# adolliou/euispice_coreg

Hardware: AMD Instinct MI355X
Metric: lag-points/sec (whole node) on 2048² grid, 60×60 CRVAL sweep; argmax-shift match (higher is better)
Workload: dtype f64; 1 GPU; headline: Carrington 'fa' 2048x2048 grid lon(200,300) lat(-20,20), 60x60 CRVAL lags arange(-30,30,1) arcsec, small 2048^2 HRIEUV-like, ref 3072^2 FSI-like, order 2, solar_r 1.004; lag_points=3600, parallelism=single GPU, no collective, resident=True, sweeps_in_flight=2, small_stored_f32=True, use_lds=True

## Files before the change

### euispice_coreg_amd/csrc/abi_sweeps.hpp

```cpp
#pragma once
namespace {
struct SweepCall {
    const coreg_lags* lags = nullptr;
    LagDims d;
    int order = 0, method = 0, sem = 0;
    long long lag_begin = 0, lag_end = 0, n_out = 0;
    double* corr_out = nullptr;
    int out_on_device = 0;
    double* out_dev = nullptr;
    long long row() const { return (long long)d.n2 * d.nc; }
    int i1_lo() const { return (int)(lag_begin / row()); }
    int i1_hi() const { return (int)((lag_end - 1) / row()); }
};

template <typename OwnChecks>
int open_sweep(coreg_handle* h, ComboRange combo, OwnChecks own_checks, const coreg_lags* lags, int order, int method,
               int sem, int64_t lag_begin, int64_t lag_end, int grid_w, int grid_h, const char* grid_what,
               double* corr_out, int out_on_device, SweepCall* call) {
    if (method != COREG_METHOD_CORRELATION && method != COREG_METHOD_RESIDUS && method != COREG_METHOD_RESIDUS_MASKED)
        return fail(h, COREG_ENOTIMPL,
                    "method must be COREG_METHOD_CORRELATION, COREG_METHOD_RESIDUS or COREG_METHOD_RESIDUS_MASKED");
    RETCHK(check_order(h, order));
    RETCHK(own_checks());
    RETCHK(check_lags(h, lags, &call->d, lag_begin, lag_end, combo));
// ... 9 lines not shown
    call->n_out = lag_end - lag_begin;
    call->corr_out = corr_out;
    call->out_on_device = out_on_device;
    return begin_sweep(h, call->n_out, corr_out, out_on_device, &call->out_dev);
}

int close_sweep(coreg_handle* h, const SweepCall& call) {
    return end_sweep(h, call.n_out, call.corr_out, call.out_on_device, call.out_dev);
}

int close_empty_sweep(coreg_handle* h, const SweepCall& call) {
    RETCHK(fill_nan(h, call.out_dev, call.n_out));
    RETCHK(fill_nan(h, h->counts.as<double>(), call.n_out));
    return close_sweep(h, call);
}

template <typename MapAt>
Geometry local_geometry(const coreg_wcs2d& target, const SweepCall& call, MapAt at) {
    const coreg_lags& l = *call.lags;
    int e1[3], e2[3];
    extreme_lags(l.crval1, call.d.n1, e1);
    extreme_lags(l.crval2, call.d.n2, e2);
    const double v1 = l.crval1[e1[1]], v2 = l.crval2[e2[1]];
    const double s1 = lag_step(l.crval1, call.d.n1), s2 = lag_step(l.crval2, call.d.n2);
    const double u = target.naxis1 * 0.5, v = target.naxis2 * 0.5;
    double x0, y0, xi, yi, xj, yj, xa, ya, xb, yb;
    Geometry g;
    if (!at(v1, v2, u, v, &x0, &y0) || !at(v1, v2, u + 1, v, &xi, &yi) || !at(v1, v2, u, v + 1, &xj, &yj) ||
        !at(v1 + s1, v2, u, v, &xa, &ya) || !at(v1, v2 + s2, u, v, &xb, &yb))
        return g;
    g.dx_di = xi - x0;
    g.dy_di = yi - y0;
    g.dx_dj = xj - x0;
    g.dy_dj = yj - y0;
    g.ax = xa - x0;
    g.ay = ya - y0;
    g.bx = xb - x0;
    g.by = yb - y0;
    return g;
}

Plan plan_sweep(coreg_handle* h, const Geometry& geo, const SweepCall& call) {
    return choose_plan(h, geo, call.i1_hi() - call.i1_lo() + 1, call.d.n2, h->opt_use_lds ? lds_window_elems(h) : (1LL << 40));
}

bool combo_slots(const SweepCall& call, const coreg_wcs2d& small, const Plan& plan, long long c, coreg_wcs2d* hc,
                 SlotList* slots) {
    const long long first = (call.lag_begin - c + call.d.nc - 1) / call.d.nc;
    if (first * call.d.nc + c >= call.lag_end) return false;
    int i3, i4, i5;
    call.d.inner(c, &i3, &i4, &i5);
    if (shift_header(small, 0.0, 0.0, call.lags->cdelt1[i3], call.lags->cdelt2[i4], call.lags->crota[i5], call.sem, hc))
        return false;
    build_slots(call.d, c, call.lag_begin, call.lag_end, plan.sw, plan.sh, slots);
    return slots->n_batches > 0;
}

template <int MODE>
int precompute(coreg_handle* h, const PrecomputeArgs& pa, int n_tiles, int n_groups, int n_batches, bool launch = true) {
    if (launch) RETCHK(launch_precompute<MODE>(h, pa, n_tiles, n_groups, n_batches));
    h->last_precompute = [pa, n_tiles, n_groups, n_batches](coreg_handle* hh) {
        return launch_precompute<MODE>(hh, pa, n_tiles, n_groups, n_batches);
    };
    return COREG_OK;
}

SweepLaunchSpec sweep_launch(const SweepCall& call, int mode, size_t slot_off, int n_batches, int n_tiles) {
    SweepLaunchSpec sl;
    sl.mode = mode;
    sl.order = call.order;
    sl.method = call.method;
    sl.slot_off = slot_off;
    sl.n_batches = n_batches;
    sl.n_tiles = n_tiles;
    sl.lag_begin = call.lag_begin;
    sl.out_dev = call.out_dev;
    return sl;
}

int finalize_pending(coreg_handle* h, const coreg_handle::PendingFinalize& pf, long long* refine_count, double* out_dev,
                     FinalizeArgs* f) {
    *f = FinalizeArgs{};
    RETCHK(fill_refine(h, &f->refine, pf.refine.mode, pf.refine.order, pf.refine.lane_params, pf.refine.car_inv,
                       pf.n_slots));
    f->refine.enabled = pf.refine.enabled;
    f->refine_count = refine_count;
    f->partials = h->sums.as<double>() + pf.slot_off;
    f->n_groups = 1;
    f->n_slots = pf.n_slots;
    f->part_stride = h->sums_slots;
    f->out_index = h->fin_outidx.as<long long>() + pf.slot_off;
    f->lag_begin = pf.lag_begin;
    f->out = out_dev;
    f->counts = h->counts.as<double>();
    f->residus = pf.residus;
    f->n_required = (long long)h->gW * h->gH;
    launch_finalize(h, *f);
    return COREG_OK;
}
}

extern "C" {
int coreg_sweep_carrington(coreg_handle* h, const coreg_wcs2d* hdr_small, const coreg_carr_grid* grid, double solar_r,
                           const coreg_lags* lags, int order, int method, int cdelt_semantics, int64_t lag_begin,
                           int64_t lag_end, double* corr_out, int out_on_device) {
    if (!h) return COREG_EINVAL;
    const ComboRange combo = take_combo_range(h);
// ... 636 lines not shown
```

### euispice_coreg_amd/csrc/coreg_hip.hip

```cpp
#include <hip/hip_runtime.h>

#include <algorithm>
#include <chrono>
#include <cmath>
#include <cstdio>
#include <cstdlib>
#include <cstring>
#include <limits>
#include <condition_variable>
#include <map>
#include <memory>
#include <mutex>
#include <string>
#include <thread>
#include <functional>
#include <type_traits>
#include <utility>
#include <vector>

#include "fit.hpp"
#include "geometry.hpp"
#include "kernels.hpp"
#include <atomic>
#include "ricecomp.hpp"
#include "riceenc.hpp"

using namespace coreg;

#define COREG_VERSION "0.1.0"

#include "host_state.hpp"
#include "host_upload.hpp"
#include "host_plan.hpp"
#include "host_fix_launch.hpp"
#include "sweep_variant.hpp"
#include "host_sweep_launch.hpp"
#include "host_fix_lists.hpp"
#include "host_sweep_io.hpp"
#include "host_context.hpp"
#include "host_pixels.hpp"


extern "C" {

const char* coreg_version(void) { return "coreg_hip " COREG_VERSION " (gfx950)"; }

int coreg_create(coreg_handle** out, int device) {
    if (!out) return COREG_EINVAL;
    *out = nullptr;
    coreg_handle* h = new (std::nothrow) coreg_handle();
    if (!h) return COREG_ENOMEM;
    int ndev = 0;
    hipError_t e = hipGetDeviceCount(&ndev);
    if (e != hipSuccess || ndev < 1) {
        delete h;
        return COREG_EHIP;
    }
    if (device < 0) {
        if (hipGetDevice(&device) != hipSuccess) device = 0;
    }
    if (device >= ndev) {
        delete h;
        return COREG_EINVAL;
    }
    h->device = device;
    if (hipSetDevice(device) != hipSuccess || hipStreamCreateWithFlags(&h->stream, hipStreamNonBlocking) != hipSuccess ||
        hipEventCreate(&h->ev_end[0]) != hipSuccess ||
        hipEventCreate(&h->ev_end[1]) != hipSuccess || hipEventRecord(h->ev_end[0], h->stream) != hipSuccess ||
        hipEventRecord(h->ev_end[1], h->stream) != hipSuccess ||
        h->pivots.reserve(2 * sizeof(double)) != hipSuccess ||
        hipMemsetAsync(h->pivots.p, 0, 2 * sizeof(double), h->stream) != hipSuccess) {
        h->own_stream = h->stream != nullptr;
        coreg_destroy(h);
        return COREG_EHIP;
    }
    h->own_stream = true;
    std::memset(&h->stats, 0, sizeof(h->stats));
    *out = h;
    return COREG_OK;
}

void coreg_destroy(coreg_handle* h) {
    if (!h) return;
// ... 164 lines not shown
```

### euispice_coreg_amd/csrc/host_plan.hpp

```cpp
#pragma once
namespace {
template <typename Fn>
void parallel_for(long long n, unsigned max_threads, long long grain, Fn fn) {
    if (n <= 0) return;
    const long long nt_max = std::max<long long>(1, std::min(max_threads, std::thread::hardware_concurrency()));
    if (grain <= 0) grain = (n + nt_max - 1) / nt_max;
    const long long nt = std::min(nt_max, (n + grain - 1) / grain);
    if (nt <= 1) {
        fn(0ll, n);
        return;
    }
    std::atomic<long long> next(0);
    auto worker = [&] {
        for (long long lo = next.fetch_add(grain); lo < n; lo = next.fetch_add(grain)) fn(lo, std::min(n, lo + grain));
    };
    std::vector<std::thread> th;
    for (long long t = 1; t < nt; ++t) th.emplace_back(worker);
    worker();
    for (auto& x : th) x.join();
}

struct LagDims {
    int n1, n2, n3, n4, n5;
    long long nc;
    long long c0;
    long long total() const { return (long long)n1 * n2 * nc; }
    void inner(long long c, int* i3, int* i4, int* i5) const {
        const long long g = c + c0;
        *i5 = (int)(g % n5);
        *i4 = (int)((g / n5) % n4);
        *i3 = (int)(g / ((long long)n5 * n4));
    }
};

struct ComboRange {
    long long begin = 0, end = 0;
};
ComboRange take_combo_range(coreg_handle* h) {
    ComboRange r;
    r.begin = h->opt_combo_begin;
    r.end = h->opt_combo_end;
    h->opt_combo_begin = h->opt_combo_end = 0;
    return r;
}
int check_lags(coreg_handle* h, const coreg_lags* l, LagDims* d, int64_t begin, int64_t end, ComboRange combo = ComboRange()) {
    if (!l || !l->crval1 || !l->crval2 || !l->cdelt1 || !l->cdelt2 || !l->crota)
        return fail(h, COREG_EINVAL, "lags: null array");
    if (l->n_crval1 < 1 || l->n_crval2 < 1 || l->n_cdelt1 < 1 || l->n_cdelt2 < 1 || l->n_crota < 1)
        return fail(h, COREG_EINVAL, "lags: every axis needs at least one value");
    d->n1 = l->n_crval1;
    d->n2 = l->n_crval2;
    d->n3 = l->n_cdelt1;
    d->n4 = l->n_cdelt2;
    d->n5 = l->n_crota;
    d->nc = (long long)d->n3 * d->n4 * d->n5;
    d->c0 = 0;
    {
        const long long cb = combo.begin, ce = combo.end;
        if (cb != 0 || ce != 0) {
            if (cb < 0 || ce <= cb || ce > d->nc)
                return fail(h, COREG_EINVAL, "combo_begin/combo_end outside [0, n_cdelt1 * n_cdelt2 * n_crota]");
            d->c0 = cb;
            d->nc = ce - cb;
        }
    }
    if (begin < 0 || end > d->total() || begin > end)
        return fail(h, COREG_EINVAL, "lag_begin/lag_end outside [0, n_lags]");
    const double* ax[5] = {l->crval1, l->crval2, l->cdelt1, l->cdelt2, l->crota};
    const int32_t na[5] = {l->n_crval1, l->n_crval2, l->n_cdelt1, l->n_cdelt2, l->n_crota};
    for (int k = 0; k < 5; ++k)
        for (int32_t i = 0; i < na[k]; ++i)
            if (!std::isfinite(ax[k][i])) return fail(h, COREG_EINVAL, "lags: a non-finite value");
    return COREG_OK;
}

static int check_wcs(coreg_handle* h, const coreg_wcs2d* w, bool carrington_transform) {
    const char* why = wcs_problem(*w, carrington_transform);
    return why ? fail(h, COREG_EINVAL, why) : COREG_OK;
}
static int check_grid(coreg_handle* h, const coreg_carr_grid* g) {
    if (g->n_lon >= 1 && g->n_lat >= 1 && too_many(g->n_lon, g->n_lat))
        return fail(h, COREG_EINVAL, "Carrington grid: more than 2^31 - 1 points");
    const char* why = grid_problem(*g);
    return why ? fail(h, COREG_EINVAL, why) : COREG_OK;
}

struct Geometry {
    double dx_di = 1, dx_dj = 0, dy_di = 0, dy_dj = 1;
    double ax = 0, ay = 0, bx = 0, by = 0;
};
struct Plan {
    int tile_w = 32;
    int sw = 16, sh = 16;
    double window = 0;
    double win_w = 0, win_h = 0;
};

Plan choose_plan(coreg_handle* h, const Geometry& g, int m1, int n2, long long lds_elems) {
    Plan best, fallback;
    double best_cost = std::numeric_limits<double>::max(), fb_win = std::numeric_limits<double>::max();
    const int sw_hi = h->opt_patch_w > 0 ? std::min<int>((int)h->opt_patch_w, kBlock) : kBlock;
    for (int tw = 4; tw <= 256; tw *= 2) {
        if (h->opt_tile_w > 0 && tw != h->opt_tile_w) continue;
        const int th = kTilePts / tw;
        if (th < 1) continue;
        const double tex = tw * std::fabs(g.dx_di) + th * std::fabs(g.dx_dj);
        const double tey = tw * std::fabs(g.dy_di) + th * std::fabs(g.dy_dj);
        for (int sw = 1; sw <= std::min(m1, sw_hi); ++sw) {
            int sh = std::min(n2, kBlock / sw);
            if (sh < 1) break;
            const int cols = (m1 + sw - 1) / sw, rows = (n2 + sh - 1) / sh;
            sh = (n2 + rows - 1) / rows;
            const int sw2 = (m1 + cols - 1) / cols;
            const double ex = tex + sw2 * std::fabs(g.ax) + sh * std::fabs(g.bx) + 6.0;
            const double ey = tey + sw2 * std::fabs(g.ay) + sh * std::fabs(g.by) + 6.0;
            const double win = (ex + 1.0) * ey;
            if (win < fb_win) {
                fb_win = win;
                fallback.tile_w = tw;
                fallback.sw = sw2;
                fallback.sh = sh;
                fallback.window = win;
                fallback.win_w = ex + 1.0;
                fallback.win_h = ey;
            }
            if (win > 0.94 * (double)lds_elems) continue;
            const double cost = (double)cols * rows * (1.0 + 0.08 * win / (double)lds_elems);
            if (cost < best_cost) {
                best_cost = cost;
                best.tile_w = tw;
                best.sw = sw2;
                best.sh = sh;
                best.window = win;
                best.win_w = ex + 1.0;
                best.win_h = ey;
            }
        }
    }
    const Plan& r = best_cost < std::numeric_limits<double>::max() ? best : fallback;
    if (std::getenv("COREG_DEBUG_PLAN"))
        std::fprintf(stderr, "[coreg plan] tile %d x %d, lag patch %d x %d, window estimate %.0f (%.1f x %.1f) of %lld elements; "
                     "geometry d/di (%.3f, %.3f) d/dj (%.3f, %.3f) lag1 (%.3f, %.3f) lag2 (%.3f, %.3f)\n", r.tile_w,
                     kTilePts / r.tile_w, r.sw, r.sh, r.window, r.win_w, r.win_h, lds_elems, g.dx_di, g.dy_di, g.dx_dj, g.dy_dj, g.ax, g.ay,
                     g.bx, g.by);
    return r;
}

void extreme_lags(const double* v, int n, int out[3]) {
    int lo = 0, hi = 0;
    for (int i = 1; i < n; ++i) {
        if (v[i] < v[lo] || v[lo] != v[lo]) lo = i;
        if (v[i] > v[hi] || v[hi] != v[hi]) hi = i;
    }
    const double mid = 0.5 * (v[lo] + v[hi]);
    int m = lo;
    for (int i = 0; i < n; ++i)
        if (std::fabs(v[i] - mid) < std::fabs(v[m] - mid)) m = i;
    out[0] = lo;
    out[1] = m;
    out[2] = hi;
}

double lag_step(const double* v, int n) {
    if (n < 2) return 0.0;
    double lo = v[0], hi = v[0];
    for (int i = 1; i < n; ++i) {
        lo = std::min(lo, v[i]);
        hi = std::max(hi, v[i]);
    }
    return (hi - lo) / (double)(n - 1);
}

struct SlotList {
    std::vector<int> i1, i2;
    std::vector<long long> outidx;
    int n_batches = 0;
};

void build_slots(const LagDims& d, long long c, long long begin, long long end, int sw, int sh, SlotList* s) {
    s->i1.clear();
    s->i2.clear();
    s->outidx.clear();
    s->n_batches = 0;
    {
        const size_t cap = (size_t)((d.n1 + sw - 1) / sw + 1) * ((d.n2 + sh - 1) / sh) * kBlock;
        s->i1.reserve(cap);
        s->i2.reserve(cap);
        s->outidx.reserve(cap);
    }
    const long long row = (long long)d.n2 * d.nc;
    const int i1_lo = (int)(begin / row);
    const int i1_hi = (int)((end - 1) / row);
    const int m1 = i1_hi - i1_lo + 1;
    for (int p1 = 0; p1 * sw < m1; ++p1)
        for (int p2 = 0; p2 * sh < d.n2; ++p2) {
            bool any = false;
            const size_t at = s->i1.size();
            for (int t = 0; t < kBlock; ++t) {
                int lx = t % sw, ly = t / sw;
                bool valid = ly < sh;
                if (!valid) lx = ly = 0;
                int i1 = i1_lo + p1 * sw + lx, i2 = p2 * sh + ly;
                if (i1 > i1_hi) {
                    i1 = i1_hi;
                    valid = false;
                }
                if (i2 > d.n2 - 1) {
                    i2 = d.n2 - 1;
                    valid = false;
                }
                const long long idx = ((long long)i1 * d.n2 + i2) * d.nc + c;
                if (idx < begin || idx >= end) valid = false;
                s->i1.push_back(i1);
                s->i2.push_back(i2);
                s->outidx.push_back(valid ? idx : -1);
                any |= valid;
            }
            if (!any) {
                s->i1.resize(at);
                s->i2.resize(at);
                s->outidx.resize(at);
            } else {
                s->n_batches++;
            }
        }
}

int pick_groups(coreg_handle* h, int n_batches, int n_tiles) {
    if (h->opt_shard_world > 1) {
        const long long per_rank = 8 * std::max<long long>(1, std::llround(256.0 / (8.0 * n_batches)));
        return (int)std::min<long long>(per_rank * h->opt_shard_world, 1000 / (8 * h->opt_shard_world) * 8 * h->opt_shard_world);
    }
    long long g = h->opt_n_groups > 0 ? h->opt_n_groups : (4096 + n_batches - 1) / n_batches;
    (void)n_tiles;
    g = std::max<long long>(8, std::min<long long>(h->opt_n_groups > 0 ? 1000 : 256, ((g + 7) / 8) * 8));
    return (int)g;
}

void pick_taper(const coreg_handle* h, int n_groups, int n_batches, int* tmin, int* tfrac) {
    *tmin = (int)h->opt_taper_min;
    if (h->opt_taper_frac >= 0) {
        *tfrac = (int)h->opt_taper_frac;
        return;
    }
    const double rounds = (double)n_groups * n_batches / 256.0;
    *tfrac = (rounds >= (double)h->opt_taper_rounds && n_groups >= 128 && h->opt_shard_world <= 1) ? 512 : 0;
}

template <int MODE>
int launch_precompute(coreg_handle* h, const PrecomputeArgs& a, int n_tiles, int n_groups, int n_batches) {
    EventPair* ev = next_event(h, h->ev_pre, h->ev_pre_used);
    if (!ev) return fail(h, COREG_EHIP, "hipEventCreate failed");
    int tmin, tfrac;
    pick_taper(h, n_groups, n_batches, &tmin, &tfrac);
    PrecomputeArgs b = a;
    b.prologue = h->pending_prologue;
    const bool with_prologue = b.prologue.src != nullptr;
    std::memset(&h->pending_prologue, 0, sizeof(h->pending_prologue));
    HIPCHK(hipEventRecord(ev->a, h->stream));
    if (h->ref_dtype == COREG_F32)
        hipLaunchKernelGGL((k_precompute<MODE, float>), dim3(n_tiles), dim3(256), 0, h->stream, b);
    else
        hipLaunchKernelGGL((k_precompute<MODE, double>), dim3(n_tiles), dim3(256), 0, h->stream, b);
    (void)with_prologue;
    hipLaunchKernelGGL(k_tile_list, dim3(1), dim3(1024), 0, h->stream, (const int*)a.tile_count, n_tiles, n_groups,
                       h->tile_list.as<int>(), h->tile_cum.as<int>(), h->group_first.as<int>(),
                       h->tile_info.as<long long>(), tmin, tfrac);
    ev->b_is_next_sweep = true;
    ev->next_sweep_index = h->ev_sweep_used;
    HIPCHK(hipGetLastError());
    return COREG_OK;
}

int reserve_tiles(coreg_handle* h, int n_tiles) {
    const size_t pts = (size_t)n_tiles * kTilePts + (size_t)(kPointGroups + 1) * kChunk;
    HIPCHK(h->pts.reserve(pts * sizeof(Pt)));
    HIPCHK(h->tile_count.reserve(n_tiles * sizeof(int)));
    HIPCHK(h->tile_list.reserve(n_tiles * sizeof(int)));
    HIPCHK(h->tile_cum.reserve((n_tiles + 1) * sizeof(int)));
    HIPCHK(h->group_first.reserve(2 * 1024 * sizeof(int) + 64));
    HIPCHK(h->tile_info.reserve(8 * sizeof(long long)));
    HIPCHK(h->tile_bbox.reserve((size_t)n_tiles * 4 * sizeof(double)));
    return COREG_OK;
}

int setup_precompute(coreg_handle* h, const Plan& plan, int method, PrecomputeArgs* a, int* n_tiles) {
    std::memset(a, 0, sizeof(*a));
    a->tile_w = plan.tile_w;
    a->tile_h = kTilePts / plan.tile_w;
    a->tiles_x = (h->gW + a->tile_w - 1) / a->tile_w;
    a->tiles_y = (h->gH + a->tile_h - 1) / a->tile_h;
    *n_tiles = a->tiles_x * a->tiles_y;
    RETCHK(reserve_tiles(h, *n_tiles));
    a->ref = h->ref.p;
    a->gw = h->gW;
    a->gh = h->gH;
    a->pivot_a = h->pivots.as<double>();
    a->pts = h->pts.as<Pt>();
    a->tile_count = h->tile_count.as<int>();
    a->tile_bbox = h->tile_bbox.as<double>();
    a->residus = method != COREG_METHOD_CORRELATION ? 1 : 0;
    return COREG_OK;
}

long long lds_window_elems(const coreg_handle* h);

int pick_pitch(const coreg_handle* h, const Plan& plan, long long lds_elems, int order = 2) {
    if (h->opt_pitch == 0 || !h->opt_use_lds) return 0;
    static const int kPitches[] = {89, 121, 153, 185, 217};
    if (h->opt_pitch > 0) {
        for (int p : kPitches)
            if (p == h->opt_pitch) return p;
        return 0;
    }
    for (int p : kPitches)
        if ((double)p >= plan.win_w + (order > 2 ? 4.0 : 2.0) &&
            (double)p * (plan.win_h + (order > 2 ? 2.0 : 0.0)) <= 0.985 * (double)lds_elems)
            return p;
    return 0;
}

}
```

### euispice_coreg_amd/csrc/host_state.hpp

```cpp
#pragma once
namespace {

struct DevBuf {
    void* p = nullptr;
    size_t cap = 0;
    hipError_t reserve(size_t bytes) {
        if (bytes <= cap) return hipSuccess;
        if (p) {
            hipError_t e = hipFree(p);
            if (e != hipSuccess) return e;
            p = nullptr;
            cap = 0;
        }
        const size_t want = bytes + bytes / 4 + 256;
        hipError_t e = hipMalloc(&p, want);
        if (e != hipSuccess) return e;
        cap = want;
        return hipSuccess;
    }
    void release() {
        if (p) (void)hipFree(p);
        p = nullptr;
        cap = 0;
    }
// ... 100 lines not shown
    std::vector<double> tabs_key;
    PinBuf pin_img[2];
    hipEvent_t ev_img[2] = {nullptr, nullptr};
    int pin_img_next = 0;
    DevBuf pts, tile_count, tile_list, tile_cum, group_first, tile_info, tile_bbox;
    DevBuf rf_fix_slab;
    DevBuf counters;
    DevBuf lane_params, out_index, partials, out_dev, tmp_img;
    DevBuf counts;
    long long counts_n = -1;
    DevBuf up_f64, up_flag;
    DevBuf up_raw;
    DevBuf rice_blob, rice_rand, dec_img;
    PrologueArgs pending_prologue = {};
    DevBuf bbox_buf;
    hipStream_t aux_stream = nullptr;
    hipStream_t up_stream = nullptr;
    hipEvent_t ev_small = nullptr, ev_main = nullptr;
    bool small_pending = false;
    DevBuf red_sum_up, red_cnt_up;
    int64_t opt_overlap_upload = 1;
    int64_t opt_tap_nan_filter = 2;
    int64_t opt_async_upload = 0;
    std::thread up_thread;
    std::mutex up_m;
    std::condition_variable up_cv;
    std::function<hipError_t()> up_job;
    bool up_has = false, up_stop = false, up_busy = false;
    hipError_t up_rc = hipSuccess;
    PinBuf pin_small[2];
    hipEvent_t ev_pin_small[2] = {nullptr, nullptr};
    int pin_small_next = 0;
    std::map<std::vector<double>, std::vector<int>> border_cache;
    std::map<std::vector<double>, std::vector<unsigned char>> flags_cache;
    DevBuf border_flags, fix_partial;
    DevBuf border_dev;
    PinBuf pin_border;
    int64_t opt_border_fix = 1;
    int64_t opt_tap_fix = 1, opt_tap_cap = 1 << 24;
    DevBuf tap_count, tap_segq, tap_list, tap_skip, tap_seg_slot, tap_seg_begin, tap_pixel, tap_xw, tap_yw;
    long long tap_last[3] = {0, 0, 0};
    int64_t opt_shard_world = 1, opt_shard_rank = 0;
    int64_t opt_combo_begin = 0, opt_combo_end = 0;
    DevBuf sums;
    long long sums_slots = 0;
    struct PendingFinalize {
        long long slot_off, n_slots, lag_begin;
        int residus;
        RefineArgs refine;
        std::function<int(coreg_handle*)> replay_precompute;
        FixLaunch fixes;
    };
    std::function<int(coreg_handle*)> last_precompute;
    DevBuf rf_flags, rf_pivots, rf_list, rf_head, rf_partial;
    std::vector<PendingFinalize> pending_fin;
    DevBuf fin_outidx;
    long long pending_n_out = 0;

    int64_t opt_crop_reference = 1;
    int64_t opt_taper_min = 128, opt_taper_frac = -1, opt_taper_rounds = 6;
    int64_t opt_use_lds = 1, opt_clean_path = 1, opt_refine = 1, opt_refine_cond_log10 = 5, opt_tile_w = 0, opt_n_groups = 0, opt_lds_bytes = (159 * 1024 * kPointGroups) / 4, opt_patch_w = 0, opt_h_series = 1, opt_h_incr = 1, opt_tile_skip = 1, opt_pitch = -1;

    coreg_stats stats;
    bool stats_pending = false;
    PinBuf pin_info;
    std::vector<EventPair> ev_sweep, ev_pre;
    size_t ev_sweep_used = 0, ev_pre_used = 0;
    hipEvent_t ev_t1 = nullptr;
    hipEvent_t ev_end[2] = {nullptr, nullptr};
    PinBuf pin_plan[2];
    int plan_slot = 0;
    bool plan_open = false;
};
```

### euispice_coreg_amd/csrc/kernels_sweep.hpp

```cpp
#pragma once
namespace coreg {
struct SweepArgs {
    const void* img;
    int W, H;
    const Pt* pts;
    const int* tile_count;
    const int* tile_list;
    const int* tile_cum;
    const int* group_first;
    long long* tile_info;
    const double* tile_bbox;
    const double* lane_params;
    long long n_slots;
    int n_batches;
    int n_groups;
    int group_lo;
    double* partials;
    const double* pivots;
    int use_lds;
    int clean_path;
    int lds_elems;
    LaunchU car_inv;
};

// ... 500 lines not shown
                    cur = nxt;
                }
            }
        }
    }
#else
    for (int c = p_begin / kChunk + pg; c < n_full; c += kPointGroups) {
        const Pt* __restrict__ q = pts + c * kChunk;
        Pt pt[kChunk];
#pragma unroll
        for (int k = 0; k < kChunk; ++k) load_pt_uniform(q + k, pt[k]);
#pragma unroll
        for (int k = 0; k < kChunk; ++k)
            point_lag<MODE, ORDER, TS, LDS, ROUND, RESID, INTERIOR, PITCH, CLEAN>(acc, win, img, pitch, ox, oy, W, H, wmax,
                                                                                  hmax, px0, py0, pxw, pyw, hm, cu, pt[k].b0,
                                                                                  pt[k].b1, pt[k].a, pt[k].pad, pivot_b);
        if constexpr (CLEAN) {
            acc.n += kChunk;
            acc.a += pt[1].pad;
            acc.aa += pt[2].pad;
        }
    }
#endif
    if (pg == n_full % kPointGroups) {
        for (int p = n_full * kChunk; p < p_end; ++p) {
            Pt pt;
            load_pt_uniform(pts + p, pt);
            point_lag<MODE, ORDER, TS, LDS, ROUND, RESID, INTERIOR, PITCH>(acc, win, img, pitch, ox, oy, W, H, wmax, hmax,
                                                                           px0, py0, pxw, pyw, hm, cu, pt.b0, pt.b1, pt.a,
                                                                           pt.pad, pivot_b);
        }
    }
}

template <int MODE, int ORDER, typename TS, bool ROUND, bool RESID, int PITCH = 0>
__global__ void __launch_bounds__(kSweepThreads) k_sweep(const SweepArgs a) {
    extern __shared__ __align__(16) unsigned char lds_raw[];
    double* lds = (double*)lds_raw;
    constexpr int kWaves = kSweepThreads / 64;
    constexpr int kLagWaves = kBlock / 64;
    __shared__ double wred2[2][kLagWaves][4];
    __shared__ int wdirty[2][kWaves];
    constexpr bool kCleanPath = MODE != MODE_CAR && !RESID && ORDER != ORDER_RT && !(ROUND && sizeof(TS) == 8);
    int visit = 0;
    int n_vis = 0, n_vis_lds = 0, n_vis_int = 0, n_vis_clean = 0;

    const int b = blockIdx.x;
    const int slot8 = b & 7;
    const int q = b >> 3;
    const int batch = q % a.n_batches;
    const int group = a.group_lo + (q / a.n_batches) * 8 + slot8;

    const int lane = threadIdx.x & 63, wave = threadIdx.x >> 6;
    const int pg = __builtin_amdgcn_readfirstlane(threadIdx.x / kBlock);
    const long long slot = (long long)batch * kBlock + (threadIdx.x % kBlock);

    double px0 = 0.0, py0 = 0.0;
    H9 hm;
#pragma unroll
    for (int k = 0; k < 9; ++k) hm.h[k] = 0.0;
    if (MODE == MODE_TRANSLATE) {
        px0 = a.lane_params[slot];
        py0 = a.lane_params[a.n_slots + slot];
    } else {
#pragma unroll
        for (int k = 0; k < 9; ++k) hm.h[k] = a.lane_params[(long long)k * a.n_slots + slot];
    }

    const bool pad_lane = MODE == MODE_TRANSLATE ? (px0 != px0) : (hm.h[8] != hm.h[8]);

    Acc acc = {0, 0.0, 0.0, 0.0, 0.0, 0.0};

    const TS* __restrict__ img = (const TS*)a.img;
    const int W = a.W, H = a.H;
    const double inf = __builtin_inf();
    const int u_lo = a.group_first[1024 + group];
    const int u_hi = a.group_first[1024 + group + 1];
    const int n_list = (int)a.tile_info[0];
    const double pivot_b = a.pivots[1];
#if defined(__HIP_DEVICE_COMPILE__)
    const unsigned win = (unsigned)(uintptr_t)(__attribute__((address_space(3))) unsigned char*)lds_raw;
#else
    const unsigned win = 0;
#endif

    for (int tl = a.group_first[group]; tl < n_list && u_lo < u_hi; ++tl) {
        const int ubase = a.tile_cum[tl];
        if (ubase >= u_hi) break;
        const int tile = a.tile_list[tl];
        const int cnt = a.tile_count[tile];
        const int p_begin = max(u_lo - ubase, 0) * kUnitPts;
        const int p_end = min((u_hi - ubase) * kUnitPts, cnt);
        if (p_begin >= p_end) continue;
        const double* bb = a.tile_bbox + (size_t)tile * 4;
        const double bx0 = bb[0], bx1 = bb[1], by0 = bb[2], by1 = bb[3];

        double mnx, mxx, mny, mxy;
        if (MODE == MODE_TRANSLATE) {
            mnx = bx0 + px0;
            mxx = bx1 + px0;
            mny = by0 + py0;
            mxy = by1 + py0;
        } else {
            mnx = inf; mxx = -inf; mny = inf; mxy = -inf;
#pragma unroll
            for (int c = 0; c < 4; ++c) {
                double cx, cy;
                apply_map<MODE>(hm, a.car_inv, (c & 1) ? bx1 : bx0, (c & 2) ? by1 : by0, cx, cy);
                mnx = fmin(mnx, cx);
                mxx = fmax(mxx, cx);
                mny = fmin(mny, cy);
                mxy = fmax(mxy, cy);
            }
            if (MODE == MODE_CAR) {
                const double margin = car_tile_margin(a.car_inv.box_c, fmax(fabs(by0), fabs(by1)) + a.car_inv.pole_sep);
                mnx -= margin;
                mxx += margin;
                mny -= margin;
                mxy += margin;
            }
        }
        for (int o = 32; o > 0; o >>= 1) {
            mnx = fmin(mnx, __shfl_xor(mnx, o));
            mxx = fmax(mxx, __shfl_xor(mxx, o));
            mny = fmin(mny, __shfl_xor(mny, o));
            mxy = fmax(mxy, __shfl_xor(mxy, o));
        }
        double(*wred)[4] = wred2[visit & 1];
        int* wdirt = wdirty[visit & 1];
        ++visit;
        if (lane == 0 && wave < kLagWaves) {
            wred[wave][0] = mnx;
            wred[wave][1] = mxx;
            wred[wave][2] = mny;
            wred[wave][3] = mxy;
        }
        __syncthreads();
        mnx = fmin(fmin(wred[0][0], wred[1][0]), fmin(wred[2][0], wred[3][0]));
        mxx = fmax(fmax(wred[0][1], wred[1][1]), fmax(wred[2][1], wred[3][1]));
        mny = fmin(fmin(wred[0][2], wred[1][2]), fmin(wred[2][2], wred[3][2]));
        mxy = fmax(fmax(wred[0][3], wred[1][3]), fmax(wred[2][3], wred[3][3]));
        if (!(mxx >= 0.0) || !(mnx <= (double)(W - 1)) || !(mxy >= 0.0) || !(mny <= (double)(H - 1))) continue;
        constexpr double kClear = 1e-9;
        const bool interior = (mnx >= kClear) & (mxx <= (double)(W - 1) - kClear) & (mny >= kClear) &
                              (mxy <= (double)(H - 1) - kClear);
        constexpr bool kWide = ORDER == ORDER_RT || ORDER > 2;
        const int ord = ORDER == ORDER_RT ? a.car_inv.order_rt : ORDER;
        const int ap_lo = kWide ? ord / 2 + 1 : 1;
        const int ap_hi = kWide ? ord - ord / 2 + 1 : 2;
        const int ox = max((int)floor(fmax(mnx, 0.0)) - ap_lo, kWide ? -ap_lo : -1);
        const int oy = max((int)floor(fmax(mny, 0.0)) - ap_lo, kWide ? -ap_lo : -1);
        const int ex = min((int)floor(fmin(mxx, (double)(W - 1))) + ap_hi, kWide ? W - 1 + ap_hi : W);
        const int ey = min((int)floor(fmin(mxy, (double)(H - 1))) + ap_hi, kWide ? H - 1 + ap_hi : H);
        const int ww = ex - ox + 1, wh = ey - oy + 1;
        int pitch = PITCH > 0 ? PITCH : (ww | 1);
        if (PITCH == 0) {
            const int r = pitch & 31;
            const int up = r < 5 ? 5 - r : ((r > 11 && r < 21) ? 21 - r : (r > 27 ? 37 - r : 0));
            if ((long long)(pitch + up) * wh <= (long long)a.lds_elems) pitch += up;
        }
        const long long need = (long long)pitch * wh;
        const bool in_lds = a.use_lds && (need <= (long long)a.lds_elems) && (PITCH == 0 || ww <= PITCH);

        const Pt* __restrict__ pts = a.pts + (size_t)tile * kTilePts;

        bool swept = false;
        ++n_vis;
        {
          if (in_lds) {
            swept = true;
            ++n_vis_lds;
#ifndef COREG_STAGE_ROWS
#define COREG_STAGE_ROWS 8
#endif
#ifndef COREG_STAGE_COLS
#define COREG_STAGE_COLS 1
#endif
            constexpr int kStage = COREG_STAGE_ROWS, kCols = COREG_STAGE_COLS;
            const double scale = ORDER == 2 ? 0.25 : 1.0;
            const int wave_u = __builtin_amdgcn_readfirstlane(wave);
            double poison = 0.0;
            for (int r0 = wave_u; r0 < wh; r0 += kWaves * kStage) {
                for (int c0 = 0; c0 < ww; c0 += 64 * kCols) {
                    int gx[kCols];
#pragma unroll
                    for (int j = 0; j < kCols; ++j) {
                        const int c = c0 + 64 * j + lane;
                        gx[j] = kWide ? mirror_far(ox + min(c, ww - 1), W) : mirror_idx(ox + min(c, ww - 1), W);
// ... 26 lines not shown
            }
            if (kCleanPath && interior) {
                const int dirty = __ballot(poison != poison) != 0ull;
                if (lane == 0) wdirt[wave] = dirty;
            }
            __syncthreads();
            bool done = false;
            if constexpr (ORDER != ORDER_RT) {
                if (interior) {
                    done = true;
                    bool clean = false;
                    if constexpr (kCleanPath) clean = a.clean_path && __ballot(wdirt[lane % kWaves] != 0) == 0ull;
                    ++n_vis_int;
                    n_vis_clean += clean ? 1 : 0;
                    if (!pad_lane) {
                        const double offx = (ORDER == 2 ? 0.5 : 0.0) - (double)(ORDER / 2 + ox);
                        const double offy = (ORDER == 2 ? 0.5 : 0.0) - (double)(ORDER / 2 + oy);
                        const double pxw = MODE == MODE_TRANSLATE ? px0 + offx : offx;
                        const double pyw = MODE == MODE_TRANSLATE ? py0 + offy : offy;
                        if (kCleanPath && clean) {
                            tile_points<MODE, ORDER, TS, true, ROUND, RESID, true, PITCH, kCleanPath>(
                                acc, win, img, pitch, ox, oy, W, H, px0, py0, pxw, pyw, hm, a.car_inv, pts, p_begin, p_end,
                                pivot_b, pg);
                        } else {
                            tile_points<MODE, ORDER, TS, true, ROUND, RESID, true, PITCH>(acc, win, img, pitch, ox, oy, W, H,
                                                                                          px0, py0, pxw, pyw, hm, a.car_inv,
                                                                                          pts, p_begin, p_end, pivot_b, pg);
                        }
                    }
                }
            }
            if (!done) {
                const double offx = ORDER == 2 ? 0.5 - (double)(1 + ox) : (ORDER == 3 ? -(double)(1 + ox) : 0.0);
                const double offy = ORDER == 2 ? 0.5 - (double)(1 + oy) : (ORDER == 3 ? -(double)(1 + oy) : 0.0);
                tile_points<MODE, ORDER, TS, true, ROUND, RESID, false, PITCH>(acc, win, img, pitch, ox, oy, W, H, px0, py0,
                                                                               offx, offy, hm, a.car_inv, pts, p_begin,
                                                                               p_end, pivot_b, pg);
            }
          }
        }
        if (!swept) {
            tile_points<MODE, ORDER, TS, false, ROUND, RESID>(acc, win, img, 0, 0, 0, W, H, px0, py0, 0.0, 0.0, hm, a.car_inv, pts,
                                                              p_begin, p_end, pivot_b, pg);
        }
    }

    if (threadIdx.x == 0) {
        atomicAdd((unsigned long long*)a.tile_info + 3, (unsigned long long)n_vis);
        atomicAdd((unsigned long long*)a.tile_info + 4, (unsigned long long)n_vis_lds);
        atomicAdd((unsigned long long*)a.tile_info + 5, (unsigned long long)n_vis_int);
        atomicAdd((unsigned long long*)a.tile_info + 6, (unsigned long long)n_vis_clean);
    }
    __syncthreads();
    const int ls = threadIdx.x % kBlock;
    if (pg > 0) {
        double* st = lds + ((size_t)(pg - 1) * kNumSums) * kBlock + ls;
        st[0] = (double)acc.n;
        st[kBlock] = acc.a;
        st[2 * kBlock] = acc.b;
        st[3 * kBlock] = acc.aa;
        st[4 * kBlock] = acc.bb;
        st[5 * kBlock] = acc.ab;
    }
    __syncthreads();
    if (pg == 0) {
        double sn = (double)acc.n, sa = acc.a, sb = acc.b, saa = acc.aa, sbb = acc.bb, sab = acc.ab;
        for (int g = 0; g < kPointGroups - 1; ++g) {
            const double* st = lds + ((size_t)g * kNumSums) * kBlock + ls;
            sn += st[0];
            sa += st[kBlock];
            sb += st[2 * kBlock];
            saa += st[3 * kBlock];
            sbb += st[4 * kBlock];
            sab += st[5 * kBlock];
        }
        double* out = a.partials + (size_t)(group - a.group_lo) * kNumSums * a.n_slots + slot;
        out[0] = sn;
        out[a.n_slots] = sa;
        out[2 * a.n_slots] = sb;
        out[3 * a.n_slots] = saa;
        out[4 * a.n_slots] = sbb;
        out[5 * a.n_slots] = sab;
    }
}

}
```

Measured before the change: 1.173 million lag-points/s.

## Plan lag patches as variable rectangles and interleave point groups across SIMDs

```diff
diff --git a/euispice_coreg_amd/csrc/abi_sweeps.hpp b/euispice_coreg_amd/csrc/abi_sweeps.hpp
--- a/euispice_coreg_amd/csrc/abi_sweeps.hpp
+++ b/euispice_coreg_amd/csrc/abi_sweeps.hpp
@@ -85,7 +85,7 @@
     call.d.inner(c, &i3, &i4, &i5);
     if (shift_header(small, 0.0, 0.0, call.lags->cdelt1[i3], call.lags->cdelt2[i4], call.lags->crota[i5], call.sem, hc))
         return false;
-    build_slots(call.d, c, call.lag_begin, call.lag_end, plan.sw, plan.sh, slots);
+    build_slots(call.d, c, call.lag_begin, call.lag_end, plan.rects, slots);
     return slots->n_batches > 0;
 }
 
diff --git a/euispice_coreg_amd/csrc/coreg_hip.hip b/euispice_coreg_amd/csrc/coreg_hip.hip
--- a/euispice_coreg_amd/csrc/coreg_hip.hip
+++ b/euispice_coreg_amd/csrc/coreg_hip.hip
@@ -29,6 +29,7 @@
 
 #define COREG_VERSION "0.1.0"
 
+#include "lag_plan.hpp"
 #include "host_state.hpp"
 #include "host_upload.hpp"
 #include "host_plan.hpp"
diff --git a/euispice_coreg_amd/csrc/host_plan.hpp b/euispice_coreg_amd/csrc/host_plan.hpp
--- a/euispice_coreg_amd/csrc/host_plan.hpp
+++ b/euispice_coreg_amd/csrc/host_plan.hpp
@@ -20,18 +20,12 @@
     for (auto& x : th) x.join();
 }
 
-struct LagDims {
-    int n1, n2, n3, n4, n5;
-    long long nc;
-    long long c0;
-    long long total() const { return (long long)n1 * n2 * nc; }
-    void inner(long long c, int* i3, int* i4, int* i5) const {
-        const long long g = c + c0;
-        *i5 = (int)(g % n5);
-        *i4 = (int)((g / n5) % n4);
-        *i3 = (int)(g / ((long long)n5 * n4));
-    }
-};
+using lag_plan::Geometry;
+using lag_plan::LagDims;
+using lag_plan::Plan;
+using lag_plan::SlotList;
+using lag_plan::build_slots;
+static_assert(lag_plan::kSlots == kBlock && lag_plan::kWaveLags == 64, "lag_plan.hpp restates the kernels' constants");
 
 struct ComboRange {
     long long begin = 0, end = 0;
@@ -85,64 +79,37 @@
     return why ? fail(h, COREG_EINVAL, why) : COREG_OK;
 }
 
-struct Geometry {
-    double dx_di = 1, dx_dj = 0, dy_di = 0, dy_dj = 1;
-    double ax = 0, ay = 0, bx = 0, by = 0;
-};
-struct Plan {
-    int tile_w = 32;
-    int sw = 16, sh = 16;
-    double window = 0;
-    double win_w = 0, win_h = 0;
-};
-
 Plan choose_plan(coreg_handle* h, const Geometry& g, int m1, int n2, long long lds_elems) {
-    Plan best, fallback;
-    double best_cost = std::numeric_limits<double>::max(), fb_win = std::numeric_limits<double>::max();
-    const int sw_hi = h->opt_patch_w > 0 ? std::min<int>((int)h->opt_patch_w, kBlock) : kBlock;
-    for (int tw = 4; tw <= 256; tw *= 2) {
-        if (h->opt_tile_w > 0 && tw != h->opt_tile_w) continue;
-        const int th = kTilePts / tw;
-        if (th < 1) continue;
-        const double tex = tw * std::fabs(g.dx_di) + th * std::fabs(g.dx_dj);
-        const double tey = tw * std::fabs(g.dy_di) + th * std::fabs(g.dy_dj);
-        for (int sw = 1; sw <= std::min(m1, sw_hi); ++sw) {
-            int sh = std::min(n2, kBlock / sw);
-            if (sh < 1) break;
-            const int cols = (m1 + sw - 1) / sw, rows = (n2 + sh - 1) / sh;
-            sh = (n2 + rows - 1) / rows;
-            const int sw2 = (m1 + cols - 1) / cols;
-            const double ex = tex + sw2 * std::fabs(g.ax) + sh * std::fabs(g.bx) + 6.0;
-            const double ey = tey + sw2 * std::fabs(g.ay) + sh * std::fabs(g.by) + 6.0;
-            const double win = (ex + 1.0) * ey;
-            if (win < fb_win) {
-                fb_win = win;
-                fallback.tile_w = tw;
-                fallback.sw = sw2;
-                fallback.sh = sh;
-                fallback.window = win;
-                fallback.win_w = ex + 1.0;
-                fallback.win_h = ey;
-            }
-            if (win > 0.94 * (double)lds_elems) continue;
-            const double cost = (double)cols * rows * (1.0 + 0.08 * win / (double)lds_elems);
-            if (cost < best_cost) {
-                best_cost = cost;
-                best.tile_w = tw;
-                best.sw = sw2;
-                best.sh = sh;
-                best.window = win;
-                best.win_w = ex + 1.0;
-                best.win_h = ey;
-            }
+    lag_plan::PlanOptions o;
+    o.tile_w = (int)h->opt_tile_w;
+    o.patch_w = (int)h->opt_patch_w;
+    coreg_handle::PlanMemo& memo = h->plan_memo;
+    const bool same = memo.valid && memo.m1 == m1 && memo.n2 == n2 && memo.lds_elems == lds_elems && memo.o.tile_w == o.tile_w &&
+                      memo.o.patch_w == o.patch_w && std::memcmp(&memo.g, &g, sizeof(g)) == 0;
+    if (!same) {
+        memo.plan = lag_plan::plan_patches(g, m1, n2, lds_elems, o, kTilePts);
+        memo.g = g;
+        memo.m1 = m1;
+        memo.n2 = n2;
+        memo.lds_elems = lds_elems;
+        memo.o = o;
+        memo.valid = true;
+    }
+    const Plan& r = memo.plan;
+    if (std::getenv("COREG_DEBUG_PLAN")) {
+        std::string patches;
+        for (size_t k = 0; k < r.rects.size(); ++k) {
+            size_t n = 1;
+            while (k + n < r.rects.size() && r.rects[k + n].w == r.rects[k].w && r.rects[k + n].h == r.rects[k].h) ++n;
+            patches += (patches.empty() ? "" : " + ") + std::to_string(n) + " of " + std::to_string(r.rects[k].w) + " x " +
+                       std::to_string(r.rects[k].h);
+            k += n - 1;
         }
-    }
-    const Plan& r = best_cost < std::numeric_limits<double>::max() ? best : fallback;
-    if (std::getenv("COREG_DEBUG_PLAN"))
-        std::fprintf(stderr, "[coreg plan] tile %d x %d, lag patch %d x %d, window estimate %.0f (%.1f x %.1f) of %lld elements; "
+        std::fprintf(stderr, "[coreg plan] tile %d x %d, lag patches %s = %d live lag-waves, window estimate %.0f (%.1f x %.1f) of %lld elements; "
                      "geometry d/di (%.3f, %.3f) d/dj (%.3f, %.3f) lag1 (%.3f, %.3f) lag2 (%.3f, %.3f)\n", r.tile_w,
-                     kTilePts / r.tile_w, r.sw, r.sh, r.window, r.win_w, r.win_h, lds_elems, g.dx_di, g.dy_di, g.dx_dj, g.dy_dj, g.ax, g.ay,
-                     g.bx, g.by);
+                     kTilePts / r.tile_w, patches.c_str(), r.live_waves, r.window, r.win_w, r.win_h, lds_elems, g.dx_di, g.dy_di,
+                     g.dx_dj, g.dy_dj, g.ax, g.ay, g.bx, g.by);
+    }
     return r;
 }
 
@@ -169,61 +136,6 @@
         hi = std::max(hi, v[i]);
     }
     return (hi - lo) / (double)(n - 1);
-}
-
-struct SlotList {
-    std::vector<int> i1, i2;
-    std::vector<long long> outidx;
-    int n_batches = 0;
-};
-
-void build_slots(const LagDims& d, long long c, long long begin, long long end, int sw, int sh, SlotList* s) {
-    s->i1.clear();
-    s->i2.clear();
-    s->outidx.clear();
-    s->n_batches = 0;
-    {
-        const size_t cap = (size_t)((d.n1 + sw - 1) / sw + 1) * ((d.n2 + sh - 1) / sh) * kBlock;
-        s->i1.reserve(cap);
-        s->i2.reserve(cap);
-        s->outidx.reserve(cap);
-    }
-    const long long row = (long long)d.n2 * d.nc;
-    const int i1_lo = (int)(begin / row);
-    const int i1_hi = (int)((end - 1) / row);
-    const int m1 = i1_hi - i1_lo + 1;
-    for (int p1 = 0; p1 * sw < m1; ++p1)
-        for (int p2 = 0; p2 * sh < d.n2; ++p2) {
-            bool any = false;
-            const size_t at = s->i1.size();
-            for (int t = 0; t < kBlock; ++t) {
-                int lx = t % sw, ly = t / sw;
-                bool valid = ly < sh;
-                if (!valid) lx = ly = 0;
-                int i1 = i1_lo + p1 * sw + lx, i2 = p2 * sh + ly;
-                if (i1 > i1_hi) {
-                    i1 = i1_hi;
-                    valid = false;
-                }
-                if (i2 > d.n2 - 1) {
-                    i2 = d.n2 - 1;
-                    valid = false;
-                }
-                const long long idx = ((long long)i1 * d.n2 + i2) * d.nc + c;
-                if (idx < begin || idx >= end) valid = false;
-                s->i1.push_back(i1);
-                s->i2.push_back(i2);
-                s->outidx.push_back(valid ? idx : -1);
-                any |= valid;
-            }
-            if (!any) {
-                s->i1.resize(at);
-                s->i2.resize(at);
-                s->outidx.resize(at);
-            } else {
-                s->n_batches++;
-            }
-        }
 }
 
 int pick_groups(coreg_handle* h, int n_batches, int n_tiles) {
@@ -307,17 +219,12 @@
 
 int pick_pitch(const coreg_handle* h, const Plan& plan, long long lds_elems, int order = 2) {
     if (h->opt_pitch == 0 || !h->opt_use_lds) return 0;
-    static const int kPitches[] = {89, 121, 153, 185, 217};
     if (h->opt_pitch > 0) {
-        for (int p : kPitches)
+        for (int p : {89, 121, 153, 185, 217})
             if (p == h->opt_pitch) return p;
         return 0;
     }
-    for (int p : kPitches)
-        if ((double)p >= plan.win_w + (order > 2 ? 4.0 : 2.0) &&
-            (double)p * (plan.win_h + (order > 2 ? 2.0 : 0.0)) <= 0.985 * (double)lds_elems)
-            return p;
-    return 0;
-}
-
-}
+    return lag_plan::pitch_for(plan, lds_elems, order);
+}
+
+}
diff --git a/euispice_coreg_amd/csrc/host_state.hpp b/euispice_coreg_amd/csrc/host_state.hpp
--- a/euispice_coreg_amd/csrc/host_state.hpp
+++ b/euispice_coreg_amd/csrc/host_state.hpp
@@ -176,6 +176,14 @@
         FixLaunch fixes;
     };
     std::function<int(coreg_handle*)> last_precompute;
+    struct PlanMemo {
+        bool valid = false;
+        lag_plan::Geometry g;
+        int m1 = 0, n2 = 0;
+        long long lds_elems = 0;
+        lag_plan::PlanOptions o;
+        lag_plan::Plan plan;
+    } plan_memo;
     DevBuf rf_flags, rf_pivots, rf_list, rf_head, rf_partial;
     std::vector<PendingFinalize> pending_fin;
     DevBuf fin_outidx;
diff --git a/euispice_coreg_amd/csrc/kernels_sweep.hpp b/euispice_coreg_amd/csrc/kernels_sweep.hpp
--- a/euispice_coreg_amd/csrc/kernels_sweep.hpp
+++ b/euispice_coreg_amd/csrc/kernels_sweep.hpp
@@ -576,8 +576,10 @@
     const int group = a.group_lo + (q / a.n_batches) * 8 + slot8;
 
     const int lane = threadIdx.x & 63, wave = threadIdx.x >> 6;
-    const int pg = __builtin_amdgcn_readfirstlane(threadIdx.x / kBlock);
-    const long long slot = (long long)batch * kBlock + (threadIdx.x % kBlock);
+    const int pg = __builtin_amdgcn_readfirstlane(wave % kPointGroups);
+    const int lw = __builtin_amdgcn_readfirstlane(wave / kPointGroups);
+    const int ls = 64 * lw + lane;
+    const long long slot = (long long)batch * kBlock + ls;
 
     double px0 = 0.0, py0 = 0.0;
     H9 hm;
@@ -653,11 +655,11 @@
         double(*wred)[4] = wred2[visit & 1];
         int* wdirt = wdirty[visit & 1];
         ++visit;
-        if (lane == 0 && wave < kLagWaves) {
-            wred[wave][0] = mnx;
-            wred[wave][1] = mxx;
-            wred[wave][2] = mny;
-            wred[wave][3] = mxy;
+        if (lane == 0 && pg == 0) {
+            wred[lw][0] = mnx;
+            wred[lw][1] = mxx;
+            wred[lw][2] = mny;
+            wred[lw][3] = mxy;
         }
         __syncthreads();
         mnx = fmin(fmin(wred[0][0], wred[1][0]), fmin(wred[2][0], wred[3][0]));
@@ -790,7 +792,6 @@
         atomicAdd((unsigned long long*)a.tile_info + 6, (unsigned long long)n_vis_clean);
     }
     __syncthreads();
-    const int ls = threadIdx.x % kBlock;
     if (pg > 0) {
         double* st = lds + ((size_t)(pg - 1) * kNumSums) * kBlock + ls;
         st[0] = (double)acc.n;
diff --git a/euispice_coreg_amd/csrc/lag_plan.hpp b/euispice_coreg_amd/csrc/lag_plan.hpp
--- /dev/null
+++ b/euispice_coreg_amd/csrc/lag_plan.hpp
@@ -0,0 +1,328 @@
+#pragma once
+#include <algorithm>
+#include <cmath>
+#include <limits>
+#include <vector>
+
+namespace lag_plan {
+constexpr int kSlots = 256;
+constexpr int kWaveLags = 64;
+
+struct LagDims {
+    int n1, n2, n3, n4, n5;
+    long long nc;
+    long long c0;
+    long long total() const { return (long long)n1 * n2 * nc; }
+    void inner(long long c, int* i3, int* i4, int* i5) const {
+        const long long g = c + c0;
+        *i5 = (int)(g % n5);
+        *i4 = (int)((g / n5) % n4);
+        *i3 = (int)(g / ((long long)n5 * n4));
+    }
+};
+
+struct Geometry {
+    double dx_di = 1, dx_dj = 0, dy_di = 0, dy_dj = 1;
+    double ax = 0, ay = 0, bx = 0, by = 0;
+};
+
+struct Rect {
+    int x0, y0, w, h;
+};
+inline int rect_waves(int w, int h) { return (w * h + kWaveLags - 1) / kWaveLags; }
+
+struct Plan {
+    int tile_w = 32;
+    std::vector<Rect> rects;
+    int live_waves = 0;
+    double window = 0;
+    double win_w = 0, win_h = 0;
+};
+
+struct PlanOptions {
+    int tile_w = 0;
+    int patch_w = 0;
+};
+
+namespace detail {
+struct TileExtent {
+    double tex, tey;
+};
+inline TileExtent tile_extent(const Geometry& g, int tw, int th) {
+    return {tw * std::fabs(g.dx_di) + th * std::fabs(g.dx_dj), tw * std::fabs(g.dy_di) + th * std::fabs(g.dy_dj)};
+}
+inline void window_of(const Geometry& g, const TileExtent& t, int w, int h, double* ww, double* wh, double* win) {
+    const double ex = t.tex + w * std::fabs(g.ax) + h * std::fabs(g.bx) + 6.0;
+    const double ey = t.tey + w * std::fabs(g.ay) + h * std::fabs(g.by) + 6.0;
+    *ww = ex + 1.0;
+    *wh = ey;
+    *win = (ex + 1.0) * ey;
+}
+inline bool fits(double win, long long lds_elems) { return win <= 0.94 * (double)lds_elems; }
+
+struct Cost {
+    int waves = 0, batches = 0, wmax = 0;
+    bool operator<(const Cost& o) const {
+        if (waves != o.waves) return waves < o.waves;
+        if (batches != o.batches) return batches < o.batches;
+        return wmax < o.wmax;
+    }
+};
+constexpr int kNever = 1 << 28;
+
+struct StripCutter {
+    std::vector<long long> f;
+    std::vector<int> from;
+    Cost cut(int w, int n, int hcap, std::vector<int>* heights) {
+        constexpr long long kInf = std::numeric_limits<long long>::max() / 2;
+        int hk[4], nk = 0;
+        long long ck[4];
+        for (int k = 1; k <= kSlots / kWaveLags; ++k) {
+            const int h = std::min(hcap, k * kWaveLags / w);
+            if (h < 1 || (nk > 0 && h == hk[nk - 1])) continue;
+            hk[nk] = h;
+            ck[nk] = ((long long)rect_waves(w, h) << 32) + 1;
+            ++nk;
+        }
+        f.resize((size_t)n + 1);
+        from.resize((size_t)n + 1);
+        f[0] = 0;
+        for (int r = 1; r <= n; ++r) {
+            long long best = kInf;
+            int bk = -1;
+            for (int k = 0; k < nk; ++k) {
+                if (hk[k] > r) break;
+                const long long c = f[(size_t)(r - hk[k])] + ck[k];
+                if (c < best) {
+                    best = c;
+                    bk = k;
+                }
+            }
+            f[(size_t)r] = best;
+            from[(size_t)r] = bk;
+        }
+        long long best = kInf;
+        int best_r = -1;
+        for (int rest = 0; rest <= std::min(hcap, n); ++rest) {
+            long long c = f[(size_t)(n - rest)];
+            if (c >= kInf) continue;
+            if (rest > 0) c += ((long long)rect_waves(w, rest) << 32) + 1;
+            if (c < best) {
+                best = c;
+                best_r = n - rest;
+            }
+        }
+        Cost out;
+        out.waves = kNever;
+        if (best_r < 0) return out;
+        out.waves = (int)(best >> 32);
+        out.batches = (int)(best & 0xffffffffll);
+        out.wmax = w;
+        if (heights) {
+            heights->clear();
+            for (int r = best_r; r > 0; r -= hk[from[(size_t)r]]) heights->push_back(hk[from[(size_t)r]]);
+            if (n - best_r > 0) heights->push_back(n - best_r);
+            std::sort(heights->begin(), heights->end(), [](int a, int b) { return a > b; });
+            for (;;) {
+                int& hi = heights->front();
+                int& lo = heights->back();
+                if (hi - lo < 2 || rect_waves(w, hi - 1) + rect_waves(w, lo + 1) > rect_waves(w, hi) + rect_waves(w, lo)) break;
+                --hi;
+                ++lo;
+                std::sort(heights->begin(), heights->end(), [](int a, int b) { return a > b; });
+            }
+        }
+        return out;
+    }
+};
+
+inline Plan single_patch_plan(const Geometry& g, int m1, int n2, long long lds_elems, const PlanOptions& o, int tile_pts) {
+    struct Pick {
+        int tile_w = 32, sw = 16, sh = 16;
+    } best, fallback;
+    double best_cost = std::numeric_limits<double>::max(), fb_win = std::numeric_limits<double>::max();
+    const int sw_hi = o.patch_w > 0 ? std::min(o.patch_w, kSlots) : kSlots;
+    for (int tw = 4; tw <= 256; tw *= 2) {
+        if (o.tile_w > 0 && tw != o.tile_w) continue;
+        const int th = tile_pts / tw;
+        if (th < 1) continue;
+        const TileExtent te = tile_extent(g, tw, th);
+        for (int sw = 1; sw <= std::min(m1, sw_hi); ++sw) {
+            int sh = std::min(n2, kSlots / sw);
+            if (sh < 1) break;
+            const int cols = (m1 + sw - 1) / sw, rows = (n2 + sh - 1) / sh;
+            sh = (n2 + rows - 1) / rows;
+            const int sw2 = (m1 + cols - 1) / cols;
+            double ww, wh, win;
+            window_of(g, te, sw2, sh, &ww, &wh, &win);
+            if (win < fb_win) {
+                fb_win = win;
+                fallback.tile_w = tw;
+                fallback.sw = sw2;
+                fallback.sh = sh;
+            }
+            if (!fits(win, lds_elems)) continue;
+            const double cost = (double)cols * rows * (1.0 + 0.08 * win / (double)lds_elems);
+            if (cost < best_cost) {
+                best_cost = cost;
+                best.tile_w = tw;
+                best.sw = sw2;
+                best.sh = sh;
+            }
+        }
+    }
+    const Pick& r = best_cost < std::numeric_limits<double>::max() ? best : fallback;
+    Plan p;
+    p.tile_w = r.tile_w;
+    for (int x0 = 0; x0 < m1; x0 += r.sw)
+        for (int y0 = 0; y0 < n2; y0 += r.sh) {
+            const Rect q = {x0, y0, std::min(r.sw, m1 - x0), std::min(r.sh, n2 - y0)};
+            p.rects.push_back(q);
+            p.live_waves += rect_waves(q.w, q.h);
+        }
+    window_of(g, tile_extent(g, r.tile_w, tile_pts / r.tile_w), r.sw, r.sh, &p.win_w, &p.win_h, &p.window);
+    return p;
+}
+}
+
+inline Plan plan_patches(const Geometry& g, int m1, int n2, long long lds_elems, const PlanOptions& o, int tile_pts) {
+    using namespace detail;
+    if (o.patch_w > 0 || m1 < 1 || n2 < 1) return single_patch_plan(g, m1, n2, lds_elems, o, tile_pts);
+    Plan best;
+    double best_cost = std::numeric_limits<double>::max();
+    int best_waves = kNever;
+    const int wmax = std::min(m1, kSlots);
+    std::vector<Cost> strip((size_t)wmax + 1), col((size_t)m1 + 1);
+    std::vector<int> hcap((size_t)wmax + 1), memo_hcap((size_t)wmax + 1, -1), pick((size_t)m1 + 1);
+    std::vector<Cost> memo((size_t)wmax + 1);
+    std::vector<int> heights;
+    StripCutter cutter;
+    for (int tw = 4; tw <= 256; tw *= 2) {
+        if (o.tile_w > 0 && tw != o.tile_w) continue;
+        const int th = tile_pts / tw;
+        if (th < 1) continue;
+        const TileExtent te = tile_extent(g, tw, th);
+        int w_fit = 0, h_prev = n2;
+        for (int w = 1; w <= wmax; ++w) {
+            int h = std::min(h_prev, kSlots / w);
+            double ww, wh, win;
+            for (; h >= 1; --h) {
+                window_of(g, te, w, h, &ww, &wh, &win);
+                if (fits(win, lds_elems)) break;
+            }
+            if (h < 1) break;
+            hcap[(size_t)w] = h_prev = h;
+            if (memo_hcap[(size_t)w] != h) {
+                memo[(size_t)w] = cutter.cut(w, n2, h, nullptr);
+                memo_hcap[(size_t)w] = h;
+            }
+            strip[(size_t)w] = memo[(size_t)w];
+            w_fit = w;
+        }
+        if (w_fit < 1) continue;
+        col[0] = Cost();
+        for (int c = 1; c <= m1; ++c) {
+            col[(size_t)c].waves = kNever;
+            for (int w = 1; w <= std::min(c, w_fit); ++w) {
+                const Cost& a = col[(size_t)(c - w)];
+                if (a.waves >= kNever) continue;
+                Cost s = {a.waves + strip[(size_t)w].waves, a.batches + strip[(size_t)w].batches, std::max(a.wmax, w)};
+                if (s < col[(size_t)c]) {
+                    col[(size_t)c] = s;
+                    pick[(size_t)c] = w;
+                }
+            }
+        }
+        const Cost& total = col[(size_t)m1];
+        if (total.waves >= kNever || total.waves > best_waves) continue;
+        Plan p;
+        p.tile_w = tw;
+        p.live_waves = total.waves;
+        std::vector<int> widths;
+        for (int c = m1; c > 0; c -= pick[(size_t)c]) widths.push_back(pick[(size_t)c]);
+        std::sort(widths.begin(), widths.end(), [](int a, int b) { return a > b; });
+        int x0 = 0;
+        for (int w : widths) {
+            cutter.cut(w, n2, hcap[(size_t)w], &heights);
+            int y0 = 0;
+            for (int h : heights) {
+                p.rects.push_back({x0, y0, w, h});
+                double ww, wh, win;
+                window_of(g, te, w, h, &ww, &wh, &win);
+                p.win_w = std::max(p.win_w, ww);
+                p.win_h = std::max(p.win_h, wh);
+                p.window = std::max(p.window, win);
+                y0 += h;
+            }
+            x0 += w;
+        }
+        const double cost = (double)total.batches * (1.0 + 0.08 * p.window / (double)lds_elems);
+        if (total.waves < best_waves || cost < best_cost) {
+            best_waves = total.waves;
+            best_cost = cost;
+            best = p;
+        }
+    }
+    if (best_waves >= kNever) return single_patch_plan(g, m1, n2, lds_elems, o, tile_pts);
+    return best;
+}
+
+struct SlotList {
+    std::vector<int> i1, i2;
+    std::vector<long long> outidx;
+    int n_batches = 0;
+    int live_waves = 0;
+};
+
+inline void build_slots(const LagDims& d, long long c, long long begin, long long end, const std::vector<Rect>& rects,
+                        SlotList* s) {
+    s->i1.clear();
+    s->i2.clear();
+    s->outidx.clear();
+    s->n_batches = 0;
+    s->live_waves = 0;
+    if (end <= begin) return;
+    s->i1.reserve(rects.size() * kSlots);
+    s->i2.reserve(rects.size() * kSlots);
+    s->outidx.reserve(rects.size() * kSlots);
+    const long long row = (long long)d.n2 * d.nc;
+    const int i1_lo = (int)(begin / row);
+    const int i1_hi = (int)((end - 1) / row);
+    auto close_batch = [s](size_t at) {
+        const size_t live = s->i1.size() - at;
+        const int p1 = s->i1[at], p2 = s->i2[at];
+        s->i1.resize(at + kSlots, p1);
+        s->i2.resize(at + kSlots, p2);
+        s->outidx.resize(at + kSlots, -1);
+        s->n_batches++;
+        s->live_waves += (int)((live + kWaveLags - 1) / kWaveLags);
+    };
+    for (const Rect& q : rects) {
+        size_t at = s->i1.size();
+        for (int ly = 0; ly < q.h; ++ly)
+            for (int lx = 0; lx < q.w; ++lx) {
+                const int i1 = i1_lo + q.x0 + lx, i2 = q.y0 + ly;
+                if (i1 > i1_hi || i2 > d.n2 - 1) continue;
+                const long long idx = ((long long)i1 * d.n2 + i2) * d.nc + c;
+                if (idx < begin || idx >= end) continue;
+                if (s->i1.size() - at == (size_t)kSlots) {
+                    close_batch(at);
+                    at = s->i1.size();
+                }
+                s->i1.push_back(i1);
+                s->i2.push_back(i2);
+                s->outidx.push_back(idx);
+            }
+        if (s->i1.size() > at) close_batch(at);
+    }
+}
+
+inline int pitch_for(const Plan& plan, long long lds_elems, int order) {
+    static const int kPitches[] = {89, 121, 153, 185, 217};
+    for (int p : kPitches)
+        if ((double)p >= plan.win_w + (order > 2 ? 4.0 : 2.0) &&
+            (double)p * (plan.win_h + (order > 2 ? 2.0 : 0.0)) <= 0.985 * (double)lds_elems)
+            return p;
+    return 0;
+}
+}
diff --git a/profiles/microbench/wave_simd.hip b/profiles/microbench/wave_simd.hip
--- /dev/null
+++ b/profiles/microbench/wave_simd.hip
@@ -0,0 +1,61 @@
+#include <hip/hip_runtime.h>
+#include <cstdio>
+#include <vector>
+
+constexpr int kThreads = 1024, kWaves = kThreads / 64;
+constexpr size_t kLdsBytes = 159 * 1024;
+
+__global__ void __launch_bounds__(kThreads) k(unsigned* out, int spin) {
+    extern __shared__ double lds[];
+    for (int i = threadIdx.x; i < 2048; i += kThreads) lds[i] = (double)i;
+    __syncthreads();
+    double s = lds[threadIdx.x];
+    for (int i = 0; i < spin; ++i) s = fma(s, 1.0000001, 1e-9);
+    const unsigned hw = __builtin_amdgcn_s_getreg(4 | (0 << 6) | (31 << 11));
+    const int wave = threadIdx.x >> 6;
+    if ((threadIdx.x & 63) == 0) out[(size_t)blockIdx.x * kWaves + wave] = s == 12345.0 ? 0u : hw;
+}
+
+int main() {
+    const int blocks = 256, launches = 8;
+    unsigned* d;
+    if (hipMalloc(&d, sizeof(unsigned) * blocks * kWaves) != hipSuccess) return 1;
+    if (hipFuncSetAttribute((const void*)k, hipFuncAttributeMaxDynamicSharedMemorySize, (int)kLdsBytes) != hipSuccess) return 1;
+    std::vector<unsigned> h((size_t)blocks * kWaves);
+    long long count[kWaves][4] = {};
+    long long n_wg = 0, n_mod4 = 0, n_div4 = 0, n_class = 0;
+    for (int l = 0; l < launches; ++l) {
+        hipLaunchKernelGGL(k, dim3(blocks), dim3(kThreads), kLdsBytes, 0, d, l % 2 ? 20000 : 200);
+        if (hipMemcpy(h.data(), d, sizeof(unsigned) * h.size(), hipMemcpyDeviceToHost) != hipSuccess) return 1;
+        for (int b = 0; b < blocks; ++b) {
+            bool mod4 = true, div4 = true, cls = true;
+            unsigned seen = 0;
+            for (int w = 0; w < kWaves; ++w) {
+                const int simd = (h[(size_t)b * kWaves + w] >> 4) & 3;
+                count[w][simd]++;
+                mod4 &= simd == (w & 3);
+                div4 &= simd == (w >> 2);
+                cls &= simd == (int)((h[(size_t)b * kWaves + (w & 3)] >> 4) & 3);
+                if (w < 4) seen |= 1u << simd;
+            }
+            ++n_wg;
+            n_mod4 += mod4;
+            n_div4 += div4;
+            n_class += cls && seen == 15u;
+            if (l == 0 && b < 4) {
+                printf("launch 0 workgroup %d: cu %u se %u | wave:simd(slot)", b, (h[(size_t)b * kWaves] >> 8) & 15,
+                       (h[(size_t)b * kWaves] >> 13) & 7);
+                for (int w = 0; w < kWaves; ++w)
+                    printf(" %d:%u(%u)", w, (h[(size_t)b * kWaves + w] >> 4) & 3, h[(size_t)b * kWaves + w] & 15);
+                printf("\n");
+            }
+        }
+    }
+    printf("wave  SIMD0  SIMD1  SIMD2  SIMD3   (%lld workgroups of %d waves, %d launches of %d)\n", n_wg, kWaves, launches, blocks);
+    for (int w = 0; w < kWaves; ++w)
+        printf("%4d %6lld %6lld %6lld %6lld\n", w, count[w][0], count[w][1], count[w][2], count[w][3]);
+    printf("workgroups with SIMD = wave mod 4 for all 16 waves: %lld; with SIMD = wave / 4: %lld\n", n_mod4, n_div4);
+    printf("workgroups whose waves w, w+4, w+8, w+12 share a SIMD, the four classes on four SIMDs: %lld of %lld\n", n_class, n_wg);
+    (void)hipFree(d);
+    return 0;
+}
```

Result: faster. 1.195 million lag-points/s, median of 6 (+1.9%).
